# gradslam/gradslam

Hardware: NVIDIA H100
Metric: PointFusion frames/sec (640x480, B=8) (higher is better)
Workload: dtype f32

## Files before the change

### gradslam_b200/_C.py

```python
import ctypes
import os

import torch

_HERE = os.path.dirname(os.path.abspath(__file__))
LIB_PATH = os.environ.get("GSX_LIB_PATH") or os.path.join(_HERE, "_lib", "libgsx.so")

c_f32p = ctypes.c_void_p
c_i32p = ctypes.c_void_p
c_i64 = ctypes.c_int64
c_int = ctypes.c_int
c_float = ctypes.c_float
c_double = ctypes.c_double
c_u32 = ctypes.c_uint32
c_vp = ctypes.c_void_p

SIGNATURES = {
    "gsx_version": (c_int, []),
    "gsx_last_error": (ctypes.c_char_p, []),
    "gsx_backproject_normals_fwd": (
        c_int, [c_vp, c_i64, c_vp, c_i64, c_vp, c_i64, c_int, c_int, c_int, c_int, c_vp, c_vp, c_vp, c_vp, c_vp]),
    "gsx_backproject_normals_bwd_scratch_bytes": (c_i64, [c_int, c_int, c_int, c_int]),
    "gsx_backproject_normals_bwd": (
        c_int, [c_vp, c_i64, c_vp, c_i64, c_vp, c_i64, c_int, c_int, c_int, c_int, c_vp, c_vp, c_vp, c_vp, c_vp, c_vp,
                c_vp, c_i64, c_vp]),
    "gsx_fusion_workspace_bytes": (c_i64, [c_int, c_int, c_int]),
    "gsx_fusion_workspace_stats_offset": (c_i64, [c_int, c_int, c_int]),
    "gsx_fusion_frame_records": (
        c_int, [c_vp, c_i64, c_vp, c_i64, c_vp, c_i64, c_vp, c_vp, c_vp, c_int, c_int, c_int, c_double, c_vp, c_vp]),
    "gsx_fusion_project_select": (
        c_int, [c_vp, c_vp, c_i64, c_i64, c_vp, c_i64, c_vp, c_i64, c_int, c_int, c_int, c_float, c_float, c_vp, c_vp]),
    "gsx_fusion_merge_append": (
        c_int, [c_vp, c_vp, c_int, c_vp, c_vp, c_i64, c_vp, c_i64, c_int, c_int, c_int, c_vp, c_vp, c_vp, c_vp]),
    "gsx_fusion_merge_append_bwd": (
        c_int, [c_vp, c_vp, c_vp, c_vp, c_int, c_i64, c_vp, c_vp, c_i64, c_vp, c_vp, c_vp, c_vp, c_int, c_int, c_int,
                c_double, c_vp, c_vp, c_vp, c_vp, c_vp, c_vp, c_vp]),
    "gsx_pointfusion_sequence_groups": (c_int, [c_int]),
    "gsx_pointfusion_sequence_workspace_bytes": (c_i64, [c_int, c_int, c_int]),
    "gsx_pointfusion_sequence_gt": (
        c_int, [c_vp, c_vp, c_vp, c_i64, c_i64, c_vp, c_vp, c_vp, c_vp, c_int, c_int, c_int, c_int, c_int, c_int,
                c_float, c_float, c_double, c_vp, c_vp, c_vp]),
    "gsx_fusion_prune_scratch_bytes": (c_i64, [c_int, c_i64]),
    "gsx_fusion_prune_unstable": (
        c_int, [c_vp, c_vp, c_vp, c_i64, c_vp, c_int, c_int, c_int, c_float, c_int, c_vp, c_vp, c_i64, c_vp]),
    "gsx_fusion_prune_unstable_bwd": (c_int, [c_vp, c_vp, c_i64, c_vp, c_vp, c_i64, c_int, c_vp, c_vp, c_vp]),
    "gsx_pointfusion_sequence_gt_prune": (
        c_int, [c_vp, c_vp, c_vp, c_i64, c_i64, c_vp, c_vp, c_vp, c_vp, c_int, c_int, c_int, c_int, c_int, c_int,
                c_float, c_float, c_double, c_vp, c_vp, c_int, c_float, c_vp, c_i64, c_vp, c_vp]),
    "gsx_debug_fail_at_frame": (None, [c_int]),
    "gsx_debug_set_k2_grid_cap": (None, [c_int]),
    "gsx_debug_set_bin_capacity": (None, [c_int]),
    "gsx_peer_export": (c_int, [c_vp, c_vp, c_vp, c_vp]),
    "gsx_peer_open": (c_int, [c_vp, c_i64, c_vp]),
    "gsx_peer_close_all": (c_int, []),
    "gsx_peer_copy_rows": (c_int, [c_vp, c_i64, c_vp, c_i64, c_i64, c_i64, c_vp]),
    "gsx_ingest_raw": (c_int, [c_vp, c_vp, c_i64, c_double, c_int, c_vp, c_vp, c_vp]),
    "gsx_ingest_calibration": (c_int, [c_vp, c_i64, c_int, c_double, c_double, c_vp, c_vp, c_int, c_int, c_vp, c_vp,
                                       c_vp]),
    "gsx_compact_scratch_bytes": (c_i64, [c_i64]),
    "gsx_compact_indices": (c_int, [c_vp, c_i64, c_vp, c_vp, c_vp, c_u32, c_vp]),
    "gsx_active_eval": (c_int, [c_vp, c_vp, c_i64, c_i64, c_vp, c_i64, c_vp, c_i64, c_int, c_int, c_int, c_vp, c_vp,
                                c_vp]),
    "gsx_similar_eval": (c_int, [c_vp, c_i64, c_vp, c_i64, c_vp, c_vp, c_int, c_int, c_int, c_float, c_float, c_vp,
                                 c_vp]),
    "gsx_unique_select": (c_int, [c_vp, c_i64, c_vp, c_i64, c_vp, c_int, c_int, c_int, c_vp, c_vp, c_vp, c_vp]),
    "gsx_records_from_table": (c_int, [c_vp, c_i64, c_i64, c_int, c_int, c_int, c_vp, c_vp]),
    "gsx_knn1_scratch_bytes": (c_i64, [c_int, c_int, c_int]),
    "gsx_icp_tgt_scratch_bytes": (c_i64, [c_int, c_i64]),
    "gsx_knn1": (c_int, [c_vp, c_vp, c_int, c_vp, c_vp, c_int, c_int, c_vp, c_vp, c_vp, c_i64, c_int, c_vp]),
    "gsx_icp_normal_eq_scratch_bytes": (c_i64, [c_int]),
    "gsx_icp_normal_eq_fwd": (c_int, [c_vp, c_int, c_vp, c_vp, c_vp, c_vp, c_vp, c_i64, c_vp]),
    "gsx_icp_normal_eq_bwd": (c_int, [c_vp, c_int, c_vp, c_vp, c_vp, c_vp, c_vp, c_vp, c_vp, c_vp]),
    "gsx_icp_normal_eq_batched_fwd": (c_int, [c_vp, c_vp, c_int, c_vp, c_vp, c_int, c_int, c_vp, c_vp, c_vp, c_i64, c_vp]),
    "gsx_icp_normal_eq_batched_bwd": (c_int, [c_vp, c_vp, c_int, c_vp, c_vp, c_int, c_int, c_vp, c_vp, c_vp, c_vp, c_vp,
                                              c_vp]),
    "gsx_icp_solve_fwd": (c_int, [c_vp, c_vp, c_int, c_vp, c_vp, c_vp]),
    "gsx_icp_solve_bwd": (c_int, [c_vp, c_vp, c_int, c_vp, c_vp, c_vp, c_vp, c_vp]),
    "gsx_icp_update_fwd": (c_int, [c_vp, c_vp, c_vp, c_vp, c_vp, c_int, c_int, c_float, c_float, c_float, c_float,
                                   c_vp, c_vp, c_vp, c_vp]),
    "gsx_icp_update_bwd": (c_int, [c_vp, c_vp, c_vp, c_vp, c_vp, c_int, c_int, c_float, c_float, c_float, c_float,
                                   c_vp, c_vp, c_vp, c_vp, c_vp, c_vp, c_vp, c_vp, c_vp]),
    "gsx_rigid_transform_fwd": (c_int, [c_vp, c_i64, c_vp, c_vp, c_vp]),
    "gsx_rigid_transform_bwd_scratch_bytes": (c_i64, [c_i64]),
    "gsx_rigid_transform_batched_fwd": (c_int, [c_vp, c_vp, c_i64, c_int, c_vp, c_vp, c_vp]),
# ... 95 lines not shown
```

### gradslam_b200/csrc/gsx_common.cuh

```cuda
#pragma once
#include <cuda_runtime.h>
#include <stdint.h>

#include <cstdio>

namespace gsx {

void set_error(const char *fmt, ...);

#define GSX_CHECK_ARG(cond, ...)   \
  do {                             \
    if (!(cond)) {                 \
      gsx::set_error(__VA_ARGS__); \
      return 1;                    \
    }                              \
  } while (0)

#define GSX_CHECK_LAUNCH(name)                                                    \
  do {                                                                            \
    cudaError_t e_ = cudaGetLastError();                                          \
    if (e_ != cudaSuccess) {                                                      \
      gsx::set_error("%s: launch failed: %s", name, cudaGetErrorString(e_));     \
      return 2;                                                                   \
    }                                                                             \
// ... 162 lines not shown
                                                         int w, int H, int W) {
  FrameSample s;
  const int wa = (w < W - 1) ? w : w - 1;
  const int ha = (h < H - 1) ? h : h - 1;
  s.d = t.c;
  const float vf = t.c > 0.0f ? 1.0f : 0.0f;
  s.v = backproject(k, (float)w, (float)h, t.c);
  const float3 a1 = backproject(k, (float)(wa + 1), (float)h, t.r);
  const float3 b1 = backproject(k, (float)w, (float)(ha + 1), t.d);
  const float3 a0 = (wa == w) ? s.v : backproject(k, (float)wa, (float)h, t.l);
  const float3 b0 = (ha == h) ? s.v : backproject(k, (float)w, (float)ha, t.u);
  const float dhx = a1.x - a0.x, dhy = a1.y - a0.y, dhz = a1.z - a0.z;
  const float dvx = b1.x - b0.x, dvy = b1.y - b0.y, dvz = b1.z - b0.z;
  s.n = normalize_masked(cross_ref(dhx, dhy, dhz, dvx, dvy, dvz), vf);
  s.gv = world_vertex(pose, s.v, s.d);
  s.gn = pose ? rotate(*pose, s.n.x, s.n.y, s.n.z) : s.n;
  return s;
}

template <bool kWantNormal>
__device__ __forceinline__ FrameSample frame_sample(const float *__restrict__ dimg, const KInv &k, const Rigid *pose,
                                                    int h, int w, int H, int W) {
  FrameSample s;
  const float dc = __ldg(dimg + h * W + w);
  s.d = dc;
  const float vf = dc > 0.0f ? 1.0f : 0.0f;
  s.v = backproject(k, (float)w, (float)h, dc);
  s.n = kWantNormal ? frame_normal(dimg, k, h, w, H, W, s.v, vf) : make_float3(0.f, 0.f, 0.f);
  s.gv = world_vertex(pose, s.v, dc);
  s.gn = (pose && kWantNormal) ? rotate(*pose, s.n.x, s.n.y, s.n.z) : s.n;
  return s;
}

__device__ __forceinline__ unsigned long long argmin_key_hi(float cc, float d2) {
  const float inv_cc = 1.0f / (cc + 1e-20f);
  unsigned int kb = __float_as_uint(inv_cc);
  kb = (kb & 0x80000000u) ? ~kb : (kb | 0x80000000u);
  const unsigned int rb = __float_as_uint(d2) | 0x80000000u;
  return ((unsigned long long)kb << 32) | rb;
}

__device__ __forceinline__ float ray_d2(const float3 &fv, float x, float y, float z) {
  const float dx = fv.x - x, dy = fv.y - y, dz = fv.z - z;
  return (dx * dx + dy * dy) + dz * dz;
}

__device__ __forceinline__ unsigned int argmin_claim(unsigned int *slot, unsigned int n) {
  return atomicCAS(slot, 0u, n + 1u);
}

__device__ __forceinline__ void argmin_settle(unsigned int *slot, unsigned int n, unsigned long long key_hi,
                                              const float3 &fv, const float *geo, unsigned int old) {
  unsigned int cur = 0u;
  while (old != cur) {
    cur = old;
    const unsigned int m = cur - 1u;
    const float4 p = __ldg(reinterpret_cast<const float4 *>(geo + (int64_t)m * kGeoW));
    const unsigned long long k = argmin_key_hi(__ldg(geo + (int64_t)m * kGeoW + 6), ray_d2(fv, p.x, p.y, p.z));
    if (k < key_hi || (k == key_hi && m <= n)) return;
    old = atomicCAS(slot, cur, n + 1u);
  }
}

struct ImageBounds {
  float u_hi, v_hi;
  int H, W;
};
inline ImageBounds image_bounds(int H, int W) { return ImageBounds{(float)(W - 0.999), (float)(H - 0.999), H, W}; }

struct LiveCamera {
  Rigid tinv;
  float k[12];
// ... 99 lines not shown
```

### gradslam_b200/csrc/gsx_fusion.cu

```cuda
#include "gsx_common.cuh"
#include "gsx_exp.cuh"
#include "gsx_fusion_ws.cuh"
#include "gsx_thresholds.h"
#include "../../include/gsx.h"

namespace gsx {

constexpr int kBlock = 256;

__device__ __forceinline__ float confidence_exp(float sq_norm, float two_sigma_sq) {
  const float x = (-sq_norm) / two_sigma_sq;
  if (!(x >= -17.0f)) return 0.0f;
  return exp_f32_via_f64(x);
}
__device__ __forceinline__ float confidence_alpha(float sq_norm, float two_sigma_sq) {
  return fminf(fmaxf(confidence_exp(sq_norm, two_sigma_sq), 1e-7f), 1.01f);
}

struct FrameRecArgs {
  const float *depth;
  int64_t depth_bstride;
  const float *K;
  int64_t K_bstride;
  const float *poses;
// ... 73 lines not shown
  }
  a.ws.win[i] = 0u;
}

int launch_frame_records(const FrameRecArgs &a, cudaStream_t stream) {
  if (a.B == 0) return 0;
  const dim3 grid((unsigned)((a.W + kRecTW - 1) / kRecTW), (unsigned)((a.H + kRecTH - 1) / kRecTH), (unsigned)a.B);
  const dim3 block(kRecTW, kRecTH);
  if (a.gv)
    k_frame_records<true><<<grid, block, 0, stream>>>(a);
  else
    k_frame_records<false><<<grid, block, 0, stream>>>(a);
  GSX_CHECK_LAUNCH("gsx_fusion_frame_records");
  return 0;
}

struct ProjectArgs {
  const float *geo;
  const int32_t *counts;
  int64_t cap;
  const float *poses;
  int64_t pose_bstride;
  const float *K;
  int64_t K_bstride;
  int B;
  ImageBounds ib;
  float dot_th;
  float d2_max;
  const float4 *nrec, *vrec;
  const FrameHeader *hdr;
  unsigned int *win;
  unsigned long long *stats;
  unsigned int *bin_count;
  uint4 *bin;
  int tiles;
  int bin_cap;
};

#ifndef GSX_K2_MINB
#define GSX_K2_MINB 5
#endif

struct MapRow {
  float4 a, b;
};
__device__ __forceinline__ MapRow load_map_row(const float *geo, int64_t n) {
  MapRow m;
  m.a = __ldg(reinterpret_cast<const float4 *>(geo + n * kGeoW));
  m.b = __ldg(reinterpret_cast<const float4 *>(geo + n * kGeoW + 4));
  return m;
}

__device__ __forceinline__ void append_candidate(unsigned int *bin_count, uint4 *bin, int bin_cap, unsigned int *win,
                                                 const float *geo, int pix, unsigned int n,
                                                 unsigned long long key_hi, const float3 &fv) {
  const int t = pix / kTilePix;
  const unsigned int grp = __match_any_sync(__activemask(), t);
  const int lane = (int)(threadIdx.x & 31), leader = __ffs(grp) - 1;
  unsigned int base = 0u;
  if (lane == leader) base = atomicAdd(bin_count + t, (unsigned int)__popc(grp));
  const unsigned int s = __shfl_sync(grp, base, leader) + (unsigned int)__popc(grp & ((1u << lane) - 1u));
  if (s < (unsigned int)bin_cap)
    bin[(int64_t)t * kBinCap + s] =
        make_uint4((unsigned int)key_hi, (unsigned int)(key_hi >> 32), n, (unsigned int)(pix - t * kTilePix));
  else
    argmin_settle(win + pix, n, key_hi, fv, geo, argmin_claim(win + pix, n));
}

template <bool kFromMaps>
__device__ __forceinline__ void select_rows(const ProjectArgs &a, const LiveCamera &s_cam, const FrameHeader &s_hdr,
                                            unsigned int *s_act, int b, int count) {
  const int P = a.ib.H * a.ib.W;
  const float *geo = a.geo + (int64_t)b * a.cap * kGeoW;
  const float4 *nrec = a.nrec + (int64_t)b * P, *vrec = a.vrec + (int64_t)b * P;
  unsigned int *win = a.win + (int64_t)b * P;
  unsigned int *bin_count = a.bin_count + (int64_t)b * a.tiles;
  uint4 *bin = a.bin + (int64_t)b * a.tiles * kBinCap;
  const int64_t stride = (int64_t)gridDim.x * kBlock;
  int64_t n = (int64_t)blockIdx.x * kBlock + threadIdx.x;
  MapRow cur = load_map_row(geo, n < count ? n : 0);
  for (; n < count; n += stride) {
    const MapRow m = cur;
    const int64_t nn = n + stride;
    if (nn < count) cur = load_map_row(geo, nn);
    const PixelHit hit = project(s_cam, a.ib, m.a.x, m.a.y, m.a.z);
    if (hit.in_frustum) {
      {
        const unsigned int am = __activemask();
        if ((int)(threadIdx.x & 31) == __ffs(am) - 1) atomicAdd(s_act + (threadIdx.x >> 5), (unsigned int)__popc(am));
      }
      const int pix = hit.h * a.ib.W + hit.w;
      float3 gn;
      float4 fv;
      frame_values<false>(s_hdr, kFromMaps, s_hdr.cam.posed ? &s_hdr.cam.pose : nullptr, nrec, vrec, hit.h, hit.w,
                          a.ib.H, a.ib.W, frame_depth(s_hdr, kFromMaps, nrec, pix), gn, fv);
      const float dot = (gn.x * m.a.w + gn.y * m.b.x) + gn.z * m.b.y;
      const float3 fv3 = make_float3(fv.x, fv.y, fv.z);
      const float d2 = ray_d2(fv3, m.a.x, m.a.y, m.a.z);
      const bool live = (d2 <= a.d2_max) && (dot > a.dot_th);
      if (live)
        append_candidate(bin_count, bin, a.bin_cap, win, geo, pix, (unsigned int)n, argmin_key_hi(m.b.z, d2), fv3);
    }
  }
}

__global__ void __launch_bounds__(kBlock, GSX_K2_MINB) k_project_select(ProjectArgs a) {
  __shared__ LiveCamera s_cam;
  __shared__ FrameHeader s_hdr;
  __shared__ unsigned int s_act[kBlock / 32];
  const int b = blockIdx.y;
  const int count = a.counts[b];
  if ((int64_t)blockIdx.x * kBlock >= count) return;
  load_live_camera(s_cam, a.poses, a.pose_bstride, a.K, a.K_bstride, b);
  load_frame_header(s_hdr, a.hdr + b);
  if (threadIdx.x < kBlock / 32) s_act[threadIdx.x] = 0u;
  __syncthreads();
  if (s_hdr.from_maps)
    select_rows<true>(a, s_cam, s_hdr, s_act, b, count);
  else
    select_rows<false>(a, s_cam, s_hdr, s_act, b, count);
  __syncthreads();
  if (threadIdx.x == 0) {
    unsigned int t = 0;
#pragma unroll
    for (int i = 0; i < kBlock / 32; ++i) t += s_act[i];
    if (t) atomicAdd(a.stats + 2 * b, (unsigned long long)t);
  }
}

#ifndef GSX_K2_CTAS_PER_SM
#define GSX_K2_CTAS_PER_SM 24
#endif

static int g_k2_grid_cap = 0;

static int g_bin_cap = -1;
static int bin_capacity() { return g_bin_cap >= 0 && g_bin_cap < kBinCap ? g_bin_cap : kBinCap; }

int launch_project_select(const ProjectArgs &args, int64_t max_count, cudaStream_t stream) {
  if (args.B == 0 || max_count <= 0) return 0;
  ProjectArgs a = args;
  a.bin_cap = bin_capacity();
  int64_t bx = (max_count + kBlock - 1) / kBlock;
  const int64_t cap_blocks = g_k2_grid_cap > 0 ? (int64_t)g_k2_grid_cap : (int64_t)kNumSMs * GSX_K2_CTAS_PER_SM;
  if (bx * a.B > cap_blocks) bx = (cap_blocks + a.B - 1) / a.B;
  if (bx < 1) bx = 1;
  k_project_select<<<dim3((unsigned)bx, (unsigned)a.B), kBlock, 0, stream>>>(a);
  GSX_CHECK_LAUNCH("gsx_fusion_project_select");
  return 0;
}

struct MergeArgs {
  float *geo, *col;
  int with_cc;
  const int32_t *counts_in;
  int32_t *counts_out;
  int64_t cap;
  const float *rgb;
  int64_t rgb_bstride;
  int B, H, W;
  Workspace ws;
  int32_t *overflow;
  int32_t *assoc;
  int bin_cap;
};

constexpr unsigned int kMergeEpoch = 1u;

#ifndef GSX_K4_MINB
#define GSX_K4_MINB 4
#endif

__device__ __forceinline__ void prefetch_l2(const float *p) { asm volatile("prefetch.global.L2 [%0];" ::"l"(p)); }

template <bool kAssoc>
__global__ void __launch_bounds__(kMB, GSX_K4_MINB) k_merge_append(MergeArgs a) {
  __shared__ int s_tile;
  __shared__ int s_warp_sums[kPix][kMB / 32];
  __shared__ int s_matched[kMB / 32];
  __shared__ int s_excl;
  __shared__ __align__(16) float s_rgb[kTilePix * 3];
  __shared__ FrameHeader s_hdr;
  __shared__ unsigned long long s_key[kTilePix];
  __shared__ unsigned int s_n[kTilePix];
  const int b = blockIdx.x % a.B;
  const int T = a.ws.tiles;
  if (threadIdx.x == 0) s_tile = (int)atomicAdd(a.ws.ticket + b, 1u);
  for (int i = threadIdx.x; i < kTilePix; i += kMB) {
    s_key[i] = ~0ull;
    s_n[i] = ~0u;
  }
  load_frame_header(s_hdr, a.ws.hdr + b);
  const int count_in = a.counts_in[b];
  __syncthreads();
  const int tile = s_tile;
  const int P = a.H * a.W;
  const int lane = threadIdx.x & 31, warp = threadIdx.x >> 5;
  const int pix0 = tile * kTilePix;
  const unsigned int *win = a.ws.win + (int64_t)b * P;
  const float4 *nrec = a.ws.nrec + (int64_t)b * P, *vrec = a.ws.vrec + (int64_t)b * P;
  const float *rgb = a.rgb + b * a.rgb_bstride + (int64_t)pix0 * 3;
  const int n_bin = (int)min(a.ws.bin_count[(int64_t)b * T + tile], (unsigned int)a.bin_cap);
  const uint4 *bin = a.ws.bin + ((int64_t)b * T + tile) * kBinCap;

  const int tile_px = min(kTilePix, P - pix0);
  if ((reinterpret_cast<uintptr_t>(rgb) & 15) == 0) {
    const int n4 = (tile_px * 3) >> 2;
    for (int i = threadIdx.x; i < n4; i += kMB)
      reinterpret_cast<float4 *>(s_rgb)[i] = __ldg(reinterpret_cast<const float4 *>(rgb) + i);
    for (int i = (n4 << 2) + threadIdx.x; i < tile_px * 3; i += kMB) s_rgb[i] = __ldg(rgb + i);
  } else {
    for (int i = threadIdx.x; i < tile_px * 3; i += kMB) s_rgb[i] = __ldg(rgb + i);
  }

  int pix[kPix];
  unsigned int slot[kPix];
  float dep[kPix];
  bool matched[kPix], is_new[kPix];
#pragma unroll
  for (int j = 0; j < kPix; ++j) {
    pix[j] = pix0 + j * kMB + threadIdx.x;
    slot[j] = 0u;
    dep[j] = 0.0f;
    if (pix[j] < P) {
      slot[j] = win[pix[j]];
      dep[j] = frame_depth(s_hdr, s_hdr.from_maps, nrec, pix[j]);
    }
  }

  static_assert(kBinCap % kMB == 0, "a bin is read in whole rounds of the CTA");
  constexpr int kRec = kBinCap / kMB;
  uint4 rec[kRec];
#pragma unroll
  for (int k = 0; k < kRec; ++k) {
    const int i = k * kMB + (int)threadIdx.x;
    if (i < n_bin) rec[k] = __ldg(bin + i);
  }
#pragma unroll
  for (int k = 0; k < kRec; ++k)
    if (k * kMB + (int)threadIdx.x < n_bin) atomicMin(s_key + rec[k].w, ((unsigned long long)rec[k].y << 32) | rec[k].x);
  __syncthreads();
#pragma unroll
  for (int k = 0; k < kRec; ++k)
    if (k * kMB + (int)threadIdx.x < n_bin &&
        (((unsigned long long)rec[k].y << 32) | rec[k].x) == s_key[rec[k].w])
      atomicMin(s_n + rec[k].w, rec[k].z);
  __syncthreads();

#pragma unroll
  for (int j = 0; j < kPix; ++j) {
    const int q = j * kMB + (int)threadIdx.x;
    const unsigned int bn = s_n[q];
    if (bn != ~0u) {
      if (slot[j] == 0u) {
        slot[j] = bn + 1u;
      } else {
        const int ph = pix[j] / a.W;
        float3 gn;
        float4 fv;
        frame_values<false>(s_hdr, s_hdr.from_maps, s_hdr.cam.posed ? &s_hdr.cam.pose : nullptr, nrec, vrec, ph,
                            pix[j] - ph * a.W, a.H, a.W, dep[j], gn, fv);
        const unsigned int m = slot[j] - 1u;
        const float4 p = *reinterpret_cast<const float4 *>(a.geo + ((int64_t)b * a.cap + m) * kGeoW);
        const unsigned long long k = argmin_key_hi(a.geo[((int64_t)b * a.cap + m) * kGeoW + 6],
                                                   ray_d2(make_float3(fv.x, fv.y, fv.z), p.x, p.y, p.z));
        if (!(k < s_key[q] || (k == s_key[q] && m < bn))) slot[j] = bn + 1u;
      }
    }
    matched[j] = a.with_cc && slot[j] != 0u;
    if (matched[j]) {
      const int64_t n = (int64_t)slot[j] - 1;
      prefetch_l2(a.geo + ((int64_t)b * a.cap + n) * kGeoW);
      prefetch_l2(a.col + ((int64_t)b * a.cap + n) * kColW);
    }
  }
  int n_matched = 0;
#pragma unroll
  for (int j = 0; j < kPix; ++j) n_matched += matched[j] ? 1 : 0;
  n_matched = __reduce_add_sync(0xffffffffu, n_matched);
  if (lane == 0) s_matched[warp] = n_matched;
  int new_off[kPix];
  const int block_total = block_offsets<kMB, kPix>(
      [&](int j) {
        is_new[j] = (pix[j] < P) && (dep[j] > 0.0f) && !matched[j];
        return is_new[j];
      },
      new_off, s_warp_sums,
      [&] {
        if (threadIdx.x == 0) {
          int t = 0;
#pragma unroll
          for (int i = 0; i < kMB / 32; ++i) t += s_matched[i];
          if (t) atomicAdd(a.ws.stats + 2 * b + 1, (unsigned long long)t);
        }
      });
  unsigned long long *state = a.ws.tile_state + (int64_t)b * T;
  if (threadIdx.x == 0) publish_tile(state, tile, T, kMergeEpoch, kTileAggregate, (unsigned)block_total);

  float *geo = a.geo + (int64_t)b * a.cap * kGeoW;
  float *col = a.col + (int64_t)b * a.cap * kColW;

  float4 fv[kPix];
  float3 fn[kPix];
#pragma unroll
  for (int j = 0; j < kPix; ++j) {
    if (matched[j] || is_new[j]) {
      const int ph = pix[j] / a.W;
      frame_values<true>(s_hdr, s_hdr.from_maps, s_hdr.cam.posed ? &s_hdr.cam.pose : nullptr, nrec, vrec, ph, pix[j] - ph * a.W, a.H, a.W, dep[j], fn[j], fv[j]);
    }
  }

  float4 g0[kPix], g1[kPix], c4[kPix];
#pragma unroll
  for (int j = 0; j < kPix; ++j) {
    if (matched[j]) {
      const int64_t n = (int64_t)slot[j] - 1;
      g0[j] = *reinterpret_cast<const float4 *>(geo + n * kGeoW);
      g1[j] = *reinterpret_cast<const float4 *>(geo + n * kGeoW + 4);
      c4[j] = *reinterpret_cast<const float4 *>(col + n * kColW);
    }
  }
#pragma unroll
  for (int j = 0; j < kPix; ++j) {
    if (matched[j]) {
      const int64_t n = (int64_t)slot[j] - 1;
      const float alpha = fv[j].w;
      const float c0 = g1[j].z;
      const float tot = c0 + alpha;
      const float inv = 1.0f / ((tot == 0.0f) ? 1.0f : tot);
      const float *fc = s_rgb + (j * kMB + (int)threadIdx.x) * 3;
      float4 o0, o1, oc;
      o0.x = ((c0 * g0[j].x) + (alpha * fv[j].x)) * inv;
      o0.y = ((c0 * g0[j].y) + (alpha * fv[j].y)) * inv;
// ... 243 lines not shown
  GSX_CHECK_ARG(B >= 0 && H >= 2 && W >= 2, "gsx_fusion_frame_records: bad extents B=%d H=%d W=%d", B, H, W);
  if (B == 0) return 0;
  GSX_CHECK_ARG(depth && workspace, "gsx_fusion_frame_records: null pointer");
  GSX_CHECK_ARG((gvertex && gnormal && vertex) || (!gvertex && !gnormal && !vertex && intrinsics),
                "gsx_fusion_frame_records: pass the three frame maps, or none of them together with the intrinsics");
  GSX_CHECK_ARG(aligned16(workspace), "gsx_fusion_frame_records: the workspace must be 16-byte aligned");
  FrameRecArgs a{depth, depth_bstride, intrinsics, K_bstride, poses, pose_bstride, gvertex, gnormal, vertex, B, H, W,
                 (float)(2.0 * (sigma * sigma)), fusion_workspace(workspace, B, H, W)};
  return launch_frame_records(a, (cudaStream_t)stream);
}

extern "C" int gsx_fusion_project_select(const float *map_geometry, const int32_t *counts, int64_t capacity,
                                         int64_t max_count, const float *poses, int64_t pose_bstride,
                                         const float *intrinsics, int64_t K_bstride, int B, int H, int W,
                                         float dist_th, float dot_th, void *workspace, void *stream) {
  GSX_CHECK_ARG(B >= 0 && H >= 2 && W >= 2, "gsx_fusion_project_select: bad extents B=%d H=%d W=%d", B, H, W);
  if (max_count <= 0 || B == 0) return 0;
  GSX_CHECK_ARG(map_geometry && counts, "gsx_fusion_project_select: null map pointer");
  GSX_CHECK_ARG(poses && intrinsics && workspace, "gsx_fusion_project_select: null frame pointer");
  GSX_CHECK_ARG(aligned16(map_geometry) && aligned16(workspace),
                "gsx_fusion_project_select: geometry rows and workspace must be 16-byte aligned");
  GSX_CHECK_ARG(max_count <= capacity, "gsx_fusion_project_select: max_count %lld > capacity %lld",
                (long long)max_count, (long long)capacity);
  const Workspace ws = fusion_workspace(workspace, B, H, W);
  ProjectArgs a{map_geometry, counts, capacity, poses, pose_bstride, intrinsics, K_bstride, B, image_bounds(H, W),
                dot_th, sqrt_lt_threshold(dist_th), ws.nrec, ws.vrec, ws.hdr, ws.win, ws.stats, ws.bin_count, ws.bin, ws.tiles, 0};
  return launch_project_select(a, max_count, (cudaStream_t)stream);
}

extern "C" void gsx_debug_set_k2_grid_cap(int ctas) { g_k2_grid_cap = ctas > 0 ? ctas : 0; }

extern "C" void gsx_debug_set_bin_capacity(int records) { g_bin_cap = records >= 0 ? records : -1; }

extern "C" int gsx_fusion_merge_append(float *map_geometry, float *map_colors, int with_ccounts,
                                       const int32_t *counts_in, int32_t *counts_out, int64_t capacity,
                                       const float *rgb, int64_t rgb_bstride, int B, int H, int W, void *workspace,
                                       int32_t *overflow_flag, int32_t *assoc_out, void *stream) {
  GSX_CHECK_ARG(B >= 0 && H >= 2 && W >= 2, "gsx_fusion_merge_append: bad extents B=%d H=%d W=%d", B, H, W);
  if (B == 0) return 0;
  GSX_CHECK_ARG(map_geometry && map_colors && counts_in && counts_out, "gsx_fusion_merge_append: null map pointer");
  GSX_CHECK_ARG(counts_in != counts_out, "gsx_fusion_merge_append: counts_in and counts_out must not alias");
  GSX_CHECK_ARG(rgb && workspace && overflow_flag, "gsx_fusion_merge_append: null frame pointer");
  GSX_CHECK_ARG(aligned16(map_geometry) && aligned16(map_colors) && aligned16(workspace),
                "gsx_fusion_merge_append: map rows and workspace must be 16-byte aligned");
  GSX_CHECK_ARG(capacity <= 0x7fffffffll, "gsx_fusion_merge_append: capacity must fit int32 (counts are int32)");
  MergeArgs a{map_geometry, map_colors, with_ccounts ? 1 : 0, counts_in, counts_out, capacity, rgb, rgb_bstride, B, H,
              W, fusion_workspace(workspace, B, H, W), overflow_flag, assoc_out, 0};
  return launch_merge_append(a, (cudaStream_t)stream);
}

extern "C" int gsx_fusion_merge_append_bwd(const int32_t *assoc, const int32_t *counts_in, const float *map_geometry,
                                           const float *map_colors, int with_ccounts, int64_t capacity_in,
                                           const float *g_geometry, const float *g_colors, int64_t capacity_out,
                                           const float *gvertex, const float *gnormal, const float *rgb,
                                           const float *vertex, int B, int H, int W, double sigma,
                                           float *d_map_geometry, float *d_map_colors, float *d_gvertex,
                                           float *d_gnormal, float *d_rgb, float *d_vertex, void *stream) {
  GSX_CHECK_ARG(B >= 0 && H >= 2 && W >= 2, "gsx_fusion_merge_append_bwd: bad extents B=%d H=%d W=%d", B, H, W);
  if (B == 0) return 0;
  GSX_CHECK_ARG(assoc && counts_in && gvertex && gnormal && rgb && vertex, "gsx_fusion_merge_append_bwd: null input");
  GSX_CHECK_ARG(d_gvertex && d_gnormal && d_rgb && d_vertex, "gsx_fusion_merge_append_bwd: null frame gradient");
  GSX_CHECK_ARG(capacity_in == 0 || (map_geometry && map_colors && d_map_geometry && d_map_colors),
                "gsx_fusion_merge_append_bwd: null map pointer");
  GSX_CHECK_ARG(aligned16(map_geometry) && aligned16(map_colors) && aligned16(g_geometry) && aligned16(g_colors) &&
                    aligned16(d_map_geometry) && aligned16(d_map_colors),
                "gsx_fusion_merge_append_bwd: map rows must be 16-byte aligned");
// ... 13 lines not shown
```

### gradslam_b200/csrc/gsx_fusion_ws.cuh

```cuda
#pragma once
#include "gsx_common.cuh"

namespace gsx {

#ifndef GSX_KPIX
#define GSX_KPIX 2
#endif
constexpr int kMB = 256;
constexpr int kPix = GSX_KPIX;
constexpr int kTilePix = kMB * kPix;

#ifndef GSX_BIN_CAP
#define GSX_BIN_CAP 1024
#endif
constexpr int kBinCap = GSX_BIN_CAP;

struct FrameHeader {
  FrameCamera cam;
  float two_sigma_sq;
  int from_maps;
  const float *depth;
};

struct Workspace {
  float4 *nrec, *vrec;
  FrameHeader *hdr;
  unsigned int *win;
  unsigned long long *tile_state;
  unsigned int *bin_count;
  uint4 *bin;
  unsigned int *ticket;
  unsigned long long *stats;
  int tiles;
};

inline Workspace fusion_workspace(void *base, int B, int H, int W, int64_t *bytes = nullptr) {
  const int64_t P = (int64_t)H * W;
  Carver c(base);
  Workspace w;
  w.tiles = (int)((P + kTilePix - 1) / kTilePix);
  w.nrec = c.take<float4>(B * P);
  w.vrec = c.take<float4>(B * P);
  w.hdr = c.take<FrameHeader>(B);
  w.win = c.take<unsigned int>(B * P);
  w.tile_state = c.take<unsigned long long>((int64_t)B * w.tiles);
  w.bin_count = c.take<unsigned int>((int64_t)B * w.tiles);
  w.bin = c.take<uint4>((int64_t)B * w.tiles * kBinCap);
  w.ticket = c.take<unsigned int>(B);
  w.stats = c.take<unsigned long long>(2 * (int64_t)B);
  if (bytes) *bytes = c.bytes;
  return w;
}

}
```

### gradslam_b200/csrc/gsx_tables.cu

```cuda
#include "gsx_common.cuh"
#include "gsx_fusion_ws.cuh"
#include "gsx_thresholds.h"
#include "../../include/gsx.h"

namespace gsx {

constexpr int kTB = 256;

struct CompactArgs {
  const uint8_t *flags;
  int64_t n;
  int64_t *out_idx;
  int64_t *out_count;
  unsigned long long *state;
  unsigned int *ticket;
  int tiles;
  unsigned int epoch;
};

__global__ void __launch_bounds__(kTB) k_compact(CompactArgs a) {
  __shared__ int s_tile, s_excl;
  __shared__ int s_warp[4][kTB / 32];
  if (threadIdx.x == 0) s_tile = draw_tile_ticket(a.ticket, a.tiles);
  __syncthreads();
// ... 33 lines not shown
  uint8_t *flags;
  int32_t *hw;
};

__global__ void __launch_bounds__(kTB) k_active_eval(ActiveArgs a) {
  __shared__ LiveCamera s_cam;
  const int b = blockIdx.y;
  load_live_camera(s_cam, a.poses, a.pose_bstride, a.K, a.K_bstride, b);
  __syncthreads();
  const int64_t n = (int64_t)blockIdx.x * kTB + threadIdx.x;
  if (n >= a.width) return;
  bool live = n < a.counts[b];
  int pix = 0;
  if (live) {
    const float4 p = __ldg(reinterpret_cast<const float4 *>(a.geo + ((int64_t)b * a.cap + n) * kGeoW));
    const PixelHit hit = project(s_cam, a.ib, p.x, p.y, p.z);
    live = hit.in_frustum;
    pix = hit.h * a.ib.W + hit.w;
  }
  a.flags[(int64_t)b * a.width + n] = live ? 1 : 0;
  a.hw[(int64_t)b * a.width + n] = pix;
}

struct RowArgs {
  const int64_t *table;
  int64_t rows;
  const float *geo;
  int64_t cap;
  const float *gv, *gn;
  int B, H, W;
  float d2_max, dot_th;
  uint8_t *flags;
  unsigned int *win;
};

__device__ __forceinline__ bool row_ok(const RowArgs &a, int64_t b, int64_t n, int64_t h, int64_t w) {
  return b >= 0 && b < a.B && n >= 0 && n < a.cap && h >= 0 && h < a.H && w >= 0 && w < a.W;
}

__global__ void __launch_bounds__(kTB) k_similar_eval(RowArgs a) {
  const int64_t r = (int64_t)blockIdx.x * kTB + threadIdx.x;
  if (r >= a.rows) return;
  const int64_t b = a.table[r * 4], n = a.table[r * 4 + 1], h = a.table[r * 4 + 2], w = a.table[r * 4 + 3];
  bool ok = row_ok(a, b, n, h, w);
  if (ok) {
    const float *p = a.geo + (b * a.cap + n) * kGeoW;
    const float *m = p + 3;
    const float *g = a.gv + ((b * a.H + h) * a.W + w) * 3;
    const float *q = a.gn + ((b * a.H + h) * a.W + w) * 3;
    const float dx = __ldg(g) - __ldg(p), dy = __ldg(g + 1) - __ldg(p + 1), dz = __ldg(g + 2) - __ldg(p + 2);
    const float d2 = (dx * dx + dy * dy) + dz * dz;
    const float dot = (__ldg(q) * __ldg(m) + __ldg(q + 1) * __ldg(m + 1)) + __ldg(q + 2) * __ldg(m + 2);
    ok = (d2 <= a.d2_max) && (dot > a.dot_th);
  }
  a.flags[r] = ok ? 1 : 0;
}

__global__ void __launch_bounds__(kTB) k_unique_select(RowArgs a) {
  const int64_t r = (int64_t)blockIdx.x * kTB + threadIdx.x;
  if (r >= a.rows) return;
  const int64_t b = a.table[r * 4], n = a.table[r * 4 + 1], h = a.table[r * 4 + 2], w = a.table[r * 4 + 3];
  if (!row_ok(a, b, n, h, w)) return;
  const float *geo = a.geo + b * a.cap * kGeoW, *p = geo + n * kGeoW;
  const float *g = a.gv + ((b * a.H + h) * a.W + w) * 3;
  const float3 fv = make_float3(__ldg(g), __ldg(g + 1), __ldg(g + 2));
  const unsigned long long key = argmin_key_hi(__ldg(p + 6), ray_d2(fv, __ldg(p), __ldg(p + 1), __ldg(p + 2)));
  unsigned int *slot = a.win + (b * a.H + h) * a.W + w;
  argmin_settle(slot, (unsigned int)n, key, fv, geo, argmin_claim(slot, (unsigned int)n));
}

__global__ void __launch_bounds__(kTB) k_records_from_table(RowArgs a) {
  const int64_t r = (int64_t)blockIdx.x * kTB + threadIdx.x;
  if (r >= a.rows) return;
  const int64_t b = a.table[r * 4], n = a.table[r * 4 + 1], h = a.table[r * 4 + 2], w = a.table[r * 4 + 3];
  if (!row_ok(a, b, n, h, w)) return;
  a.win[(b * a.H + h) * a.W + w] = (unsigned int)n + 1u;
}

__global__ void __launch_bounds__(kTB) k_unique_emit(const unsigned int *win, int64_t pixels, uint8_t *flags,
                                                     int64_t *n_out) {
  const int64_t i = (int64_t)blockIdx.x * kTB + threadIdx.x;
  if (i >= pixels) return;
  const unsigned int v = win[i];
  flags[i] = v != 0u ? 1 : 0;
  n_out[i] = (int64_t)v - 1;
}

}

using namespace gsx;

static inline int64_t tb_blocks(int64_t n) { return (n + kTB - 1) / kTB; }

extern "C" int64_t gsx_compact_scratch_bytes(int64_t n) {
  if (n < 0) return -1;
  const int64_t tiles = (n + kTB * 4 - 1) / (kTB * 4);
  return (tiles + 1) * 8 + 256;
}

extern "C" int gsx_compact_indices(const uint8_t *flags, int64_t n, int64_t *out_idx, int64_t *out_count,
                                   void *scratch, uint32_t epoch, void *stream) {
  GSX_CHECK_ARG(out_count && scratch, "gsx_compact_indices: null pointer");
  GSX_CHECK_ARG(n >= 0 && n < (1ll << 31) * 1024, "gsx_compact_indices: bad n");
  GSX_CHECK_ARG(epoch >= 1 && epoch < (1u << 30), "gsx_compact_indices: epoch out of range");
  cudaStream_t s = (cudaStream_t)stream;
  if (n == 0) {
    cudaMemsetAsync(out_count, 0, 8, s);
    return 0;
  }
// ... 27 lines not shown
  GSX_CHECK_ARG(table && map_geometry && gvertex && gnormal && flags, "gsx_similar_eval: null pointer");
  RowArgs a{table, rows, map_geometry, capacity, gvertex, gnormal, B, H, W, sqrt_lt_threshold(dist_th), dot_th, flags,
            nullptr};
  k_similar_eval<<<(unsigned)tb_blocks(rows), kTB, 0, (cudaStream_t)stream>>>(a);
  GSX_CHECK_LAUNCH("gsx_similar_eval");
  return 0;
}

extern "C" int gsx_unique_select(const int64_t *table, int64_t rows, const float *map_geometry, int64_t capacity,
                                 const float *gvertex, int B, int H, int W, void *records, uint8_t *pixel_flags,
                                 int64_t *pixel_n, void *stream) {
  GSX_CHECK_ARG(records && pixel_flags && pixel_n, "gsx_unique_select: null pointer");
  GSX_CHECK_ARG((reinterpret_cast<uintptr_t>(records) & 3) == 0, "gsx_unique_select: records must be 4-byte aligned");
  GSX_CHECK_ARG(capacity <= 0x7fffffffll, "gsx_unique_select: capacity must fit int32");
  cudaStream_t s = (cudaStream_t)stream;
  const int64_t pixels = (int64_t)B * H * W;
  cudaMemsetAsync(records, 0, (size_t)pixels * 4, s);
  if (rows > 0) {
    GSX_CHECK_ARG(table && map_geometry && gvertex, "gsx_unique_select: null pointer");
    RowArgs a{table, rows, map_geometry, capacity, gvertex, nullptr, B, H, W, 0.f, 0.f, nullptr,
              (unsigned int *)records};
    k_unique_select<<<(unsigned)tb_blocks(rows), kTB, 0, s>>>(a);
  }
  k_unique_emit<<<(unsigned)tb_blocks(pixels), kTB, 0, s>>>((const unsigned int *)records, pixels, pixel_flags, pixel_n);
  GSX_CHECK_LAUNCH("gsx_unique_select");
  return 0;
}

extern "C" int gsx_records_from_table(const int64_t *table, int64_t rows, int64_t capacity, int B, int H, int W,
                                      void *workspace, void *stream) {
  if (rows == 0) return 0;
  GSX_CHECK_ARG(table && workspace, "gsx_records_from_table: null pointer");
  GSX_CHECK_ARG(capacity <= 0x7fffffffll, "gsx_records_from_table: capacity must fit int32");
  RowArgs a{table, rows, nullptr, capacity, nullptr, nullptr, B, H, W, 0.f, 0.f, nullptr,
            fusion_workspace(workspace, B, H, W).win};
  k_records_from_table<<<(unsigned)tb_blocks(rows), kTB, 0, (cudaStream_t)stream>>>(a);
  GSX_CHECK_LAUNCH("gsx_records_from_table");
  return 0;
}
```

### include/gsx.h

```cpp
#ifndef GSX_H_
#define GSX_H_

#include <stdint.h>

#ifdef __cplusplus
extern "C" {
#endif

#define GSX_VERSION 200

int gsx_version(void);
const char *gsx_last_error(void);

int gsx_backproject_normals_fwd(const float *depth, int64_t depth_bstride, const float *intrinsics,
                                int64_t K_bstride, const float *poses, int64_t pose_bstride, int B, int L,
                                int H, int W, float *vertex, float *normal, float *gvertex, float *gnormal,
                                void *stream);

int64_t gsx_backproject_normals_bwd_scratch_bytes(int B, int L, int H, int W);
int gsx_backproject_normals_bwd(const float *depth, int64_t depth_bstride, const float *intrinsics,
                                int64_t K_bstride, const float *poses, int64_t pose_bstride, int B, int L,
                                int H, int W, const float *g_vertex, const float *g_normal,
                                const float *g_gvertex, const float *g_gnormal, float *g_depth,
                                float *g_poses, void *scratch, int64_t scratch_bytes, void *stream);
// ... 12 lines not shown
int gsx_fusion_merge_append(float *map_geometry, float *map_colors, int with_ccounts, const int32_t *counts_in,
                            int32_t *counts_out, int64_t capacity, const float *rgb, int64_t rgb_bstride, int B, int H,
                            int W, void *workspace, int32_t *overflow_flag, int32_t *assoc_out, void *stream);

int gsx_fusion_merge_append_bwd(const int32_t *assoc, const int32_t *counts_in, const float *map_geometry,
                                const float *map_colors, int with_ccounts, int64_t capacity_in,
                                const float *g_geometry, const float *g_colors, int64_t capacity_out,
                                const float *gvertex, const float *gnormal, const float *rgb, const float *vertex,
                                int B, int H, int W, double sigma, float *d_map_geometry, float *d_map_colors,
                                float *d_gvertex, float *d_gnormal, float *d_rgb, float *d_vertex, void *stream);

int gsx_pointfusion_sequence_groups(int B);
int64_t gsx_pointfusion_sequence_workspace_bytes(int B, int H, int W);
int gsx_pointfusion_sequence_gt(float *map_geometry, float *map_colors, int32_t *counts, int64_t capacity,
                                int64_t max_count0, const float *depth, const float *rgb, const float *intrinsics,
                                const float *poses, int B, int L, int s_begin, int s_end, int H, int W, float dist_th,
                                float dot_th, double sigma, void *workspace, int32_t *overflow_flag, void *stream);
int64_t gsx_fusion_prune_scratch_bytes(int B, int64_t capacity);
int gsx_fusion_prune_unstable(float *map_geometry, float *map_colors, int32_t *counts, int64_t capacity, int32_t *ring,
                              int ring_len, int step, int t_max, float c_stable, int B, int32_t *keep_map,
                              void *scratch, int64_t scratch_bytes, void *stream);
int gsx_fusion_prune_unstable_bwd(const int32_t *keep_map, const int32_t *counts_in, int64_t capacity_in,
                                  const float *g_geometry, const float *g_colors, int64_t capacity_out, int B,
                                  float *d_map_geometry, float *d_map_colors, void *stream);
int gsx_pointfusion_sequence_gt_prune(float *map_geometry, float *map_colors, int32_t *counts, int64_t capacity,
                                      int64_t max_count0, const float *depth, const float *rgb, const float *intrinsics,
                                      const float *poses, int B, int L, int s_begin, int s_end, int H, int W,
                                      float dist_th, float dot_th, double sigma, void *workspace, int32_t *ring,
                                      int t_max, float c_stable, void *prune_scratch, int64_t prune_scratch_bytes,
                                      int32_t *overflow_flag, void *stream);
void gsx_debug_fail_at_frame(int s);
void gsx_debug_set_k2_grid_cap(int ctas);
void gsx_debug_set_bin_capacity(int records);

#define GSX_IPC_HANDLE_BYTES 64
int gsx_peer_export(const void *ptr, unsigned char *handle , int64_t *offset,
                    int64_t *allocation_bytes );
int gsx_peer_open(const unsigned char *handle, int64_t offset, void **ptr_out);
int gsx_peer_close_all(void);
int gsx_peer_copy_rows(void *dst, int64_t dst_pitch_bytes, const void *src, int64_t src_pitch_bytes,
                       int64_t width_bytes, int64_t n_blocks, void *stream);

int gsx_ingest_raw(const uint8_t *rgb_u8, const uint16_t *depth_u16, int64_t n_pixels, double depth_scaling_factor,
                   int normalize_color, float *rgb_out, float *depth_out, void *stream);

int gsx_ingest_calibration(const float *intrinsics, int64_t n_intrinsics, int intrinsics_dim, double h_ratio,
                           double w_ratio, float *intrinsics_out, const float *poses, int B, int L, float *poses_out,
                           int32_t *singular_flag, void *stream);


int64_t gsx_compact_scratch_bytes(int64_t n);
int gsx_compact_indices(const uint8_t *flags, int64_t n, int64_t *out_idx, int64_t *out_count, void *scratch,
                        uint32_t epoch, void *stream);

int gsx_active_eval(const float *map_geometry, const int32_t *counts, int64_t capacity, int64_t width,
                    const float *poses, int64_t pose_bstride, const float *intrinsics, int64_t K_bstride, int B,
                    int H, int W, uint8_t *flags, int32_t *hw, void *stream);

int gsx_similar_eval(const int64_t *table, int64_t rows, const float *map_geometry, int64_t capacity,
                     const float *gvertex, const float *gnormal, int B, int H, int W, float dist_th, float dot_th,
                     uint8_t *flags, void *stream);

int gsx_unique_select(const int64_t *table, int64_t rows, const float *map_geometry, int64_t capacity,
                      const float *gvertex, int B, int H, int W, void *records, uint8_t *pixel_flags,
                      int64_t *pixel_n, void *stream);

// ... 91 lines not shown
```

Baseline: 30170.

## Pack bin records into 8 bytes and skip slot reads for untouched tiles

Bin candidate records shrink from uint4 to uint2. Each record now holds only the high key word, plus the row index and tile pixel offset packed into one word. Exact ties on the high key are settled in a separate merge pass that recomputes ray distances. A flag bit in bin_count marks tiles where any candidate fell back to the global argmin slot, so the merge kernel reads win[] only when that bit is set. This is meant to halve bin traffic and avoid per-pixel slot loads, at the cost of extra tie-handling code and two key recomputations when a bin winner meets an existing slot.

```diff
diff --git a/gradslam_b200/_C.py b/gradslam_b200/_C.py
--- a/gradslam_b200/_C.py
+++ b/gradslam_b200/_C.py
@@ -50,6 +50,7 @@
     "gsx_debug_fail_at_frame": (None, [c_int]),
     "gsx_debug_set_k2_grid_cap": (None, [c_int]),
     "gsx_debug_set_bin_capacity": (None, [c_int]),
+    "gsx_debug_set_bin_row_limit": (None, [c_i64]),
     "gsx_peer_export": (c_int, [c_vp, c_vp, c_vp, c_vp]),
     "gsx_peer_open": (c_int, [c_vp, c_i64, c_vp]),
     "gsx_peer_close_all": (c_int, []),
diff --git a/gradslam_b200/csrc/gsx_common.cuh b/gradslam_b200/csrc/gsx_common.cuh
--- a/gradslam_b200/csrc/gsx_common.cuh
+++ b/gradslam_b200/csrc/gsx_common.cuh
@@ -218,12 +218,12 @@
   return s;
 }
 
+__device__ __forceinline__ unsigned int argmin_key_lo(float d2) { return __float_as_uint(d2) | 0x80000000u; }
 __device__ __forceinline__ unsigned long long argmin_key_hi(float cc, float d2) {
   const float inv_cc = 1.0f / (cc + 1e-20f);
   unsigned int kb = __float_as_uint(inv_cc);
   kb = (kb & 0x80000000u) ? ~kb : (kb | 0x80000000u);
-  const unsigned int rb = __float_as_uint(d2) | 0x80000000u;
-  return ((unsigned long long)kb << 32) | rb;
+  return ((unsigned long long)kb << 32) | argmin_key_lo(d2);
 }
 
 __device__ __forceinline__ float ray_d2(const float3 &fv, float x, float y, float z) {
diff --git a/gradslam_b200/csrc/gsx_fusion.cu b/gradslam_b200/csrc/gsx_fusion.cu
--- a/gradslam_b200/csrc/gsx_fusion.cu
+++ b/gradslam_b200/csrc/gsx_fusion.cu
@@ -129,9 +129,10 @@
   unsigned int *win;
   unsigned long long *stats;
   unsigned int *bin_count;
-  uint4 *bin;
+  uint2 *bin;
   int tiles;
   int bin_cap;
+  unsigned int bin_rows;
 };
 
 #ifndef GSX_K2_MINB
@@ -148,18 +149,20 @@
   return m;
 }
 
-__device__ __forceinline__ void append_candidate(unsigned int *bin_count, uint4 *bin, int bin_cap, unsigned int *win,
-                                                 const float *geo, int pix, unsigned int n,
-                                                 unsigned long long key_hi, const float3 &fv) {
+__device__ __forceinline__ void append_candidate(unsigned int *bin_count, uint2 *bin, int bin_cap,
+                                                 unsigned int bin_rows, unsigned int *win, const float *geo, int pix,
+                                                 unsigned int n, unsigned long long key_hi, const float3 &fv) {
   const int t = pix / kTilePix;
-  const unsigned int grp = __match_any_sync(__activemask(), t);
+  const bool fits = n < bin_rows;
+  const unsigned int grp = __match_any_sync(__activemask(), fits ? t : ~t);
   const int lane = (int)(threadIdx.x & 31), leader = __ffs(grp) - 1;
   unsigned int base = 0u;
-  if (lane == leader) base = atomicAdd(bin_count + t, (unsigned int)__popc(grp));
-  const unsigned int s = __shfl_sync(grp, base, leader) + (unsigned int)__popc(grp & ((1u << lane) - 1u));
-  if (s < (unsigned int)bin_cap)
-    bin[(int64_t)t * kBinCap + s] =
-        make_uint4((unsigned int)key_hi, (unsigned int)(key_hi >> 32), n, (unsigned int)(pix - t * kTilePix));
+  if (lane == leader)
+    base = fits ? atomicAdd(bin_count + t, (unsigned int)__popc(grp)) : atomicOr(bin_count + t, kSlotFlag);
+  const unsigned int s =
+      (__shfl_sync(grp, base, leader) & ~kSlotFlag) + (unsigned int)__popc(grp & ((1u << lane) - 1u));
+  if (fits && s < (unsigned int)bin_cap)
+    bin[(int64_t)t * kBinCap + s] = bin_record((unsigned int)(key_hi >> 32), n, pix - t * kTilePix);
   else
     argmin_settle(win + pix, n, key_hi, fv, geo, argmin_claim(win + pix, n));
 }
@@ -169,10 +172,10 @@
                                             unsigned int *s_act, int b, int count) {
   const int P = a.ib.H * a.ib.W;
   const float *geo = a.geo + (int64_t)b * a.cap * kGeoW;
-  const float4 *nrec = a.nrec + (int64_t)b * P, *vrec = a.vrec + (int64_t)b * P;
+  const float4 *nrec = a.nrec + b * P, *vrec = a.vrec + b * P;
   unsigned int *win = a.win + (int64_t)b * P;
   unsigned int *bin_count = a.bin_count + (int64_t)b * a.tiles;
-  uint4 *bin = a.bin + (int64_t)b * a.tiles * kBinCap;
+  uint2 *bin = a.bin + (int64_t)b * a.tiles * kBinCap;
   const int64_t stride = (int64_t)gridDim.x * kBlock;
   int64_t n = (int64_t)blockIdx.x * kBlock + threadIdx.x;
   MapRow cur = load_map_row(geo, n < count ? n : 0);
@@ -196,7 +199,8 @@
       const float d2 = ray_d2(fv3, m.a.x, m.a.y, m.a.z);
       const bool live = (d2 <= a.d2_max) && (dot > a.dot_th);
       if (live)
-        append_candidate(bin_count, bin, a.bin_cap, win, geo, pix, (unsigned int)n, argmin_key_hi(m.b.z, d2), fv3);
+        append_candidate(bin_count, bin, a.bin_cap, a.bin_rows, win, geo, pix, (unsigned int)n,
+                         argmin_key_hi(m.b.z, d2), fv3);
     }
   }
 }
@@ -234,10 +238,16 @@
 static int g_bin_cap = -1;
 static int bin_capacity() { return g_bin_cap >= 0 && g_bin_cap < kBinCap ? g_bin_cap : kBinCap; }
 
+static int64_t g_bin_rows = -1;
+static unsigned int bin_row_limit() {
+  return g_bin_rows >= 0 && g_bin_rows < (int64_t)kBinRows ? (unsigned int)g_bin_rows : kBinRows;
+}
+
 int launch_project_select(const ProjectArgs &args, int64_t max_count, cudaStream_t stream) {
   if (args.B == 0 || max_count <= 0) return 0;
   ProjectArgs a = args;
   a.bin_cap = bin_capacity();
+  a.bin_rows = bin_row_limit();
   int64_t bx = (max_count + kBlock - 1) / kBlock;
   const int64_t cap_blocks = g_k2_grid_cap > 0 ? (int64_t)g_k2_grid_cap : (int64_t)kNumSMs * GSX_K2_CTAS_PER_SM;
   if (bx * a.B > cap_blocks) bx = (cap_blocks + a.B - 1) / a.B;
@@ -278,14 +288,17 @@
   __shared__ int s_excl;
   __shared__ __align__(16) float s_rgb[kTilePix * 3];
   __shared__ FrameHeader s_hdr;
+  __shared__ unsigned int s_w[kTilePix];
+  __shared__ unsigned int s_n[kTilePix];
+  __shared__ float s_fv[3][kTilePix];
   __shared__ unsigned long long s_key[kTilePix];
-  __shared__ unsigned int s_n[kTilePix];
+  constexpr unsigned int kNone = ~0u, kTied = ~0u - 1u;
   const int b = blockIdx.x % a.B;
   const int T = a.ws.tiles;
   if (threadIdx.x == 0) s_tile = (int)atomicAdd(a.ws.ticket + b, 1u);
   for (int i = threadIdx.x; i < kTilePix; i += kMB) {
-    s_key[i] = ~0ull;
-    s_n[i] = ~0u;
+    s_w[i] = ~0u;
+    s_n[i] = kNone;
   }
   load_frame_header(s_hdr, a.ws.hdr + b);
   const int count_in = a.counts_in[b];
@@ -297,8 +310,12 @@
   const unsigned int *win = a.ws.win + (int64_t)b * P;
   const float4 *nrec = a.ws.nrec + (int64_t)b * P, *vrec = a.ws.vrec + (int64_t)b * P;
   const float *rgb = a.rgb + b * a.rgb_bstride + (int64_t)pix0 * 3;
-  const int n_bin = (int)min(a.ws.bin_count[(int64_t)b * T + tile], (unsigned int)a.bin_cap);
-  const uint4 *bin = a.ws.bin + ((int64_t)b * T + tile) * kBinCap;
+  float *geo = a.geo + (int64_t)b * a.cap * kGeoW;
+  float *col = a.col + (int64_t)b * a.cap * kColW;
+  const unsigned int bin_count = a.ws.bin_count[(int64_t)b * T + tile];
+  const int n_bin = (int)min(bin_count & ~kSlotFlag, (unsigned int)a.bin_cap);
+  const bool read_slots = (bin_count & kSlotFlag) || (bin_count & ~kSlotFlag) > (unsigned int)a.bin_cap;
+  const uint2 *bin = a.ws.bin + ((int64_t)b * T + tile) * kBinCap;
 
   const int tile_px = min(kTilePix, P - pix0);
   if ((reinterpret_cast<uintptr_t>(rgb) & 15) == 0) {
@@ -320,14 +337,14 @@
     slot[j] = 0u;
     dep[j] = 0.0f;
     if (pix[j] < P) {
-      slot[j] = win[pix[j]];
+      if (read_slots) slot[j] = win[pix[j]];
       dep[j] = frame_depth(s_hdr, s_hdr.from_maps, nrec, pix[j]);
     }
   }
 
   static_assert(kBinCap % kMB == 0, "a bin is read in whole rounds of the CTA");
   constexpr int kRec = kBinCap / kMB;
-  uint4 rec[kRec];
+  uint2 rec[kRec];
 #pragma unroll
   for (int k = 0; k < kRec; ++k) {
     const int i = k * kMB + (int)threadIdx.x;
@@ -335,20 +352,53 @@
   }
 #pragma unroll
   for (int k = 0; k < kRec; ++k)
-    if (k * kMB + (int)threadIdx.x < n_bin) atomicMin(s_key + rec[k].w, ((unsigned long long)rec[k].y << 32) | rec[k].x);
+    if (k * kMB + (int)threadIdx.x < n_bin) atomicMin(s_w + bin_offset(rec[k]), rec[k].x);
   __syncthreads();
-#pragma unroll
-  for (int k = 0; k < kRec; ++k)
-    if (k * kMB + (int)threadIdx.x < n_bin &&
-        (((unsigned long long)rec[k].y << 32) | rec[k].x) == s_key[rec[k].w])
-      atomicMin(s_n + rec[k].w, rec[k].z);
-  __syncthreads();
+  bool tie = false;
+#pragma unroll
+  for (int k = 0; k < kRec; ++k) {
+    const int o = bin_offset(rec[k]);
+    if (k * kMB + (int)threadIdx.x < n_bin && rec[k].x == s_w[o] && atomicCAS(s_n + o, kNone, bin_row(rec[k])) != kNone) {
+      atomicExch(s_n + o, kTied);
+      tie = true;
+    }
+  }
+  if (__syncthreads_or(tie)) {
+#pragma unroll
+    for (int j = 0; j < kPix; ++j) {
+      const int q = j * kMB + (int)threadIdx.x;
+      if (s_n[q] == kTied) {
+        const int ph = pix[j] / a.W;
+        float3 gn;
+        float4 fv;
+        frame_values<false>(s_hdr, s_hdr.from_maps, s_hdr.cam.posed ? &s_hdr.cam.pose : nullptr, nrec, vrec, ph,
+                            pix[j] - ph * a.W, a.H, a.W, dep[j], gn, fv);
+        s_fv[0][q] = fv.x;
+        s_fv[1][q] = fv.y;
+        s_fv[2][q] = fv.z;
+        s_key[q] = ~0ull;
+      }
+    }
+    __syncthreads();
+#pragma unroll
+    for (int k = 0; k < kRec; ++k) {
+      const int o = bin_offset(rec[k]);
+      if (k * kMB + (int)threadIdx.x < n_bin && rec[k].x == s_w[o] && s_n[o] == kTied) {
+        const unsigned int n = bin_row(rec[k]);
+        const float4 p = *reinterpret_cast<const float4 *>(geo + (int64_t)n * kGeoW);
+        const float d2 = ray_d2(make_float3(s_fv[0][o], s_fv[1][o], s_fv[2][o]), p.x, p.y, p.z);
+        atomicMin(s_key + o, ((unsigned long long)argmin_key_lo(d2) << 32) | n);
+      }
+    }
+    __syncthreads();
+  }
 
 #pragma unroll
   for (int j = 0; j < kPix; ++j) {
     const int q = j * kMB + (int)threadIdx.x;
-    const unsigned int bn = s_n[q];
-    if (bn != ~0u) {
+    unsigned int bn = s_n[q];
+    if (bn == kTied) bn = (unsigned int)s_key[q];
+    if (bn != kNone) {
       if (slot[j] == 0u) {
         slot[j] = bn + 1u;
       } else {
@@ -357,11 +407,13 @@
         float4 fv;
         frame_values<false>(s_hdr, s_hdr.from_maps, s_hdr.cam.posed ? &s_hdr.cam.pose : nullptr, nrec, vrec, ph,
                             pix[j] - ph * a.W, a.H, a.W, dep[j], gn, fv);
+        const float3 fv3 = make_float3(fv.x, fv.y, fv.z);
         const unsigned int m = slot[j] - 1u;
-        const float4 p = *reinterpret_cast<const float4 *>(a.geo + ((int64_t)b * a.cap + m) * kGeoW);
-        const unsigned long long k = argmin_key_hi(a.geo[((int64_t)b * a.cap + m) * kGeoW + 6],
-                                                   ray_d2(make_float3(fv.x, fv.y, fv.z), p.x, p.y, p.z));
-        if (!(k < s_key[q] || (k == s_key[q] && m < bn))) slot[j] = bn + 1u;
+        const float4 p = *reinterpret_cast<const float4 *>(geo + (int64_t)m * kGeoW);
+        const unsigned long long k = argmin_key_hi(geo[(int64_t)m * kGeoW + 6], ray_d2(fv3, p.x, p.y, p.z));
+        const float4 pb = *reinterpret_cast<const float4 *>(geo + (int64_t)bn * kGeoW);
+        const unsigned long long kb = argmin_key_hi(geo[(int64_t)bn * kGeoW + 6], ray_d2(fv3, pb.x, pb.y, pb.z));
+        if (!(k < kb || (k == kb && m < bn))) slot[j] = bn + 1u;
       }
     }
     matched[j] = a.with_cc && slot[j] != 0u;
@@ -393,9 +445,6 @@
       });
   unsigned long long *state = a.ws.tile_state + (int64_t)b * T;
   if (threadIdx.x == 0) publish_tile(state, tile, T, kMergeEpoch, kTileAggregate, (unsigned)block_total);
-
-  float *geo = a.geo + (int64_t)b * a.cap * kGeoW;
-  float *col = a.col + (int64_t)b * a.cap * kColW;
 
   float4 fv[kPix];
   float3 fn[kPix];
@@ -705,6 +754,8 @@
 
 extern "C" void gsx_debug_set_bin_capacity(int records) { g_bin_cap = records >= 0 ? records : -1; }
 
+extern "C" void gsx_debug_set_bin_row_limit(int64_t rows) { g_bin_rows = rows >= 0 ? rows : -1; }
+
 extern "C" int gsx_fusion_merge_append(float *map_geometry, float *map_colors, int with_ccounts,
                                        const int32_t *counts_in, int32_t *counts_out, int64_t capacity,
                                        const float *rgb, int64_t rgb_bstride, int B, int H, int W, void *workspace,
diff --git a/gradslam_b200/csrc/gsx_fusion_ws.cuh b/gradslam_b200/csrc/gsx_fusion_ws.cuh
--- a/gradslam_b200/csrc/gsx_fusion_ws.cuh
+++ b/gradslam_b200/csrc/gsx_fusion_ws.cuh
@@ -15,6 +15,18 @@
 #endif
 constexpr int kBinCap = GSX_BIN_CAP;
 
+constexpr int log2_exact(int x) { return x <= 1 ? 0 : 1 + log2_exact(x / 2); }
+static_assert((kTilePix & (kTilePix - 1)) == 0, "the pixel offset of a bin record needs a power-of-two tile");
+constexpr int kOffBits = log2_exact(kTilePix);
+constexpr unsigned int kBinRows = 1u << (32 - kOffBits);
+__device__ __forceinline__ uint2 bin_record(unsigned int key_word, unsigned int n, int off) {
+  return make_uint2(key_word, (n << kOffBits) | (unsigned int)off);
+}
+__device__ __forceinline__ unsigned int bin_row(const uint2 &r) { return r.y >> kOffBits; }
+__device__ __forceinline__ int bin_offset(const uint2 &r) { return (int)(r.y & (unsigned int)(kTilePix - 1)); }
+
+constexpr unsigned int kSlotFlag = 0x80000000u;
+
 struct FrameHeader {
   FrameCamera cam;
   float two_sigma_sq;
@@ -28,7 +40,7 @@
   unsigned int *win;
   unsigned long long *tile_state;
   unsigned int *bin_count;
-  uint4 *bin;
+  uint2 *bin;
   unsigned int *ticket;
   unsigned long long *stats;
   int tiles;
@@ -45,7 +57,7 @@
   w.win = c.take<unsigned int>(B * P);
   w.tile_state = c.take<unsigned long long>((int64_t)B * w.tiles);
   w.bin_count = c.take<unsigned int>((int64_t)B * w.tiles);
-  w.bin = c.take<uint4>((int64_t)B * w.tiles * kBinCap);
+  w.bin = c.take<uint2>((int64_t)B * w.tiles * kBinCap);
   w.ticket = c.take<unsigned int>(B);
   w.stats = c.take<unsigned long long>(2 * (int64_t)B);
   if (bytes) *bytes = c.bytes;
diff --git a/gradslam_b200/csrc/gsx_tables.cu b/gradslam_b200/csrc/gsx_tables.cu
--- a/gradslam_b200/csrc/gsx_tables.cu
+++ b/gradslam_b200/csrc/gsx_tables.cu
@@ -89,6 +89,8 @@
   float d2_max, dot_th;
   uint8_t *flags;
   unsigned int *win;
+  unsigned int *bin_count;
+  int tiles;
 };
 
 __device__ __forceinline__ bool row_ok(const RowArgs &a, int64_t b, int64_t n, int64_t h, int64_t w) {
@@ -132,6 +134,7 @@
   const int64_t b = a.table[r * 4], n = a.table[r * 4 + 1], h = a.table[r * 4 + 2], w = a.table[r * 4 + 3];
   if (!row_ok(a, b, n, h, w)) return;
   a.win[(b * a.H + h) * a.W + w] = (unsigned int)n + 1u;
+  atomicOr(a.bin_count + b * a.tiles + (h * a.W + w) / kTilePix, kSlotFlag);
 }
 
 __global__ void __launch_bounds__(kTB) k_unique_emit(const unsigned int *win, int64_t pixels, uint8_t *flags,
@@ -225,8 +228,9 @@
   if (rows == 0) return 0;
   GSX_CHECK_ARG(table && workspace, "gsx_records_from_table: null pointer");
   GSX_CHECK_ARG(capacity <= 0x7fffffffll, "gsx_records_from_table: capacity must fit int32");
-  RowArgs a{table, rows, nullptr, capacity, nullptr, nullptr, B, H, W, 0.f, 0.f, nullptr,
-            fusion_workspace(workspace, B, H, W).win};
+  const Workspace ws = fusion_workspace(workspace, B, H, W);
+  RowArgs a{table, rows, nullptr, capacity, nullptr, nullptr, B, H, W, 0.f, 0.f, nullptr, ws.win, ws.bin_count,
+            ws.tiles};
   k_records_from_table<<<(unsigned)tb_blocks(rows), kTB, 0, (cudaStream_t)stream>>>(a);
   GSX_CHECK_LAUNCH("gsx_records_from_table");
   return 0;
diff --git a/include/gsx.h b/include/gsx.h
--- a/include/gsx.h
+++ b/include/gsx.h
@@ -68,6 +68,7 @@
 void gsx_debug_fail_at_frame(int s);
 void gsx_debug_set_k2_grid_cap(int ctas);
 void gsx_debug_set_bin_capacity(int records);
+void gsx_debug_set_bin_row_limit(int64_t rows);
 
 #define GSX_IPC_HANDLE_BYTES 64
 int gsx_peer_export(const void *ptr, unsigned char *handle , int64_t *offset,
```

Result: faster. 31020 (median of 6 runs) (+2.8%).
